# Hi-FT/ERD

Measured on AMD Instinct MI355X. Metric: images/sec GFL-R50 40+40 incre step @1333x800, higher is better.
Workload: dtype f32; 1 GPU; gfl_r50_fpn first_40_incre_last_40 ERD (BASELINE configs[1]), 1333x800 padded to 800x1344, fp32, procedural weights; batch_per_gpu=4, global_batch=4, parallelism=dp1

## Files before the change

erd_amd/_lib.py:

```python
from __future__ import annotations

import ctypes as C
import os

_HERE = os.path.dirname(os.path.abspath(__file__))
LIB_PATH = os.environ.get("ERD_HIP_LIB") or os.path.join(_HERE, "lib", "liberd_hip.so")

ERD_MAX_SEG = 5
ERD_MAX_TAPS = 9
ERD_MAX_GROUPS = 8
ERD_SQNORM_PARTS = 1024

c_float_p = C.c_void_p
i64 = C.c_int64
i32 = C.c_int
f32 = C.c_float


class ConvSeg(C.Structure):
    _fields_ = [("inp", C.c_void_p), ("out", C.c_void_p), ("res", C.c_void_p), ("alpha", C.c_void_p),
                ("mask", C.c_void_p), ("N", i32), ("IH", i32), ("IW", i32), ("GH", i32), ("GW", i32), ("OH", i32), ("OW", i32),
                ("in_nstride", i64), ("out_nstride", i64), ("res_nstride", i64),
                ("tap0", i32), ("ntaps", i32), ("oy", i32), ("ox", i32)]

# ... 64 lines not shown
    "erd_to_bf16": [P, P, i64, P],
    "erd_split3": [P, P, i64, P],
    "erd_conv_thin_enable": [i32],
    "erd_conv_thin_ok": [C.POINTER(ConvDesc)],
    "erd_weight_transpose_x3": [P, P, P, i32, i32, i32, i32, P],
    "erd_wino_weights_elems": [i32, i32],
    "erd_wino_weights": [P, P, i32, i32, i32, P],
    "erd_wino_conv3x3": [P, i32, P, i32, i32, P, P, i32, P, i32, P, P],
    "erd_wino_weights_x3_elems": [i32, i32],
    "erd_wino_weights_x3": [P, P, i32, i32, i32, P],
    "erd_wino_conv3x3_x3": [P, i32, P, i32, i32, P, P, i32, P, i32, P, P],
    "erd_wino_x3_couts_per_item": [P, i32, i32],
    "erd_wino_conv3x3_x3_gn": [P, i32, P, i32, i32, P, P, i32, P, P, C.c_size_t, P],
    "erd_wino_gn_finalize": [P, i32, i32, P, P, f32, P],
    "erd_wino_x3_gn_ws_bytes": [P, i32, i32],
    "erd_conv_wgrad": [C.POINTER(WgradDesc), P],
    "erd_wgrad_row3_slices": [C.POINTER(WgradDesc)],
    "erd_conv_grouped_fwd": [C.POINTER(ConvGroupedDesc), P],
    "erd_conv_grouped_dgrad": [C.POINTER(ConvGroupedDesc), P],
    "erd_conv_grouped_wgrad": [P, P, P, i32, i32, i32, i32, i32, i32, i32, P],
    "erd_conv_grouped_wgrad_splits": [i32, i32, i32, i32, i32, i32],
    "erd_deform_cols": [P, P, P, i32, i32, i32, i32, i32, P],
    "erd_deform_cols_bwd": [P, P, P, P, P, i32, i32, i32, i32, i32, P],
    "erd_wgrad_reduce": [P, i32, i32, i32, P, P, P, i32, P, P],
    "erd_wgrad_reduce_rows": [P, i32, i32, i32, i32, P, i32, P],
    "erd_wgrad_reduce_grouped": [P, i32, i32, i32, C.POINTER(WgradReduceGroups), i32, P],
    "erd_conv_wgrad_wino": [C.POINTER(WgradDesc), P],
    "erd_conv_wgrad_wino_ok": [C.POINTER(WgradDesc)],
    "erd_conv_wgrad_wino_tile": [C.POINTER(WgradDesc)],
    "erd_wgrad_wino_reduce": [P, i32, i32, i32, P, i32, P],
# ... 106 lines not shown
```

erd_amd/csrc/elementwise.hip:

```cpp
#include "erd_common.h"
#include <vector>

namespace erd {
thread_local char g_err[512] = "";
void set_error(const char* fmt, ...) {
    va_list ap;
    va_start(ap, fmt);
    vsnprintf(g_err, sizeof(g_err), fmt, ap);
    va_end(ap);
}
}

extern "C" int erd_abi_version(void) { return ERD_ABI_VERSION; }
#ifndef ERD_CSRC_SHA
#define ERD_CSRC_SHA "unknown"
#endif
extern "C" const char* erd_csrc_sha(void) { return ERD_CSRC_SHA; }
extern "C" __attribute__((weak)) int erd_probe_build_marker;
extern "C" int erd_probe_build(void) { return &erd_probe_build_marker != nullptr ? erd_probe_build_marker : 0; }
extern "C" const char* erd_last_error(void) { return erd::g_err; }
namespace erd {
static int g_cu_reserve = 0;
int usable_cus(int physical) { return physical - g_cu_reserve >= 8 ? physical - g_cu_reserve : (physical < 8 ? physical : 8); }
}
// ... 350 lines not shown
                                                       const float* __restrict__ gamma, const float* __restrict__ beta,
                                                       const float* __restrict__ mean_rstd, int64_t A, erd_levels lv,
                                                       GnChunks ch) {
    const int n = blockIdx.y;
    int s; int64_t r0, r1;
    gn_chunk(lv, ch, blockIdx.x, s, r0, r1);
    const int c4 = threadIdx.x & 63, rl = threadIdx.x >> 6;
    const int g = c4 >> 1;
    const float2 mr = *reinterpret_cast<const float2*>(mean_rstd + (((int64_t)n * lv.nseg + s) * G + g) * 2);
    const float4 ga = reinterpret_cast<const float4*>(gamma)[c4];
    const float4 be = reinterpret_cast<const float4*>(beta)[c4];
    for (int64_t r = r0 + rl; r < r1; r += 4) {
        const int64_t off = ((int64_t)n * A + r) * C + c4 * 4;
        const float4 v = erd::ld4(c + off);
        float4 o;
        o.x = fmaxf((v.x - mr.x) * mr.y * ga.x + be.x, 0.f);
        o.y = fmaxf((v.y - mr.x) * mr.y * ga.y + be.y, 0.f);
        o.z = fmaxf((v.z - mr.x) * mr.y * ga.z + be.z, 0.f);
        o.w = fmaxf((v.w - mr.x) * mr.y * ga.w + be.w, 0.f);
        erd::st4(y + off, o);
    }
}

template <int C, int G, typename T>
__global__ __launch_bounds__(256) void gn_bwd_stats_kernel(const T* __restrict__ c, const T* __restrict__ dy,
                                                           const float* __restrict__ gamma,
                                                           const float* __restrict__ beta,
                                                           const float* __restrict__ mean_rstd,
                                                           double* __restrict__ stats, float* __restrict__ dgamma,
                                                           float* __restrict__ dbeta, int64_t A, erd_levels lv,
                                                           GnChunks ch) {
    const int n = blockIdx.y;
    int s; int64_t r0, r1;
    gn_chunk(lv, ch, blockIdx.x, s, r0, r1, GN_STAT_ROWS);
// ... 844 lines not shown
```

erd_amd/csrc/erd_common.h:

```cpp
#pragma once
#include <hip/hip_runtime.h>
#include <stdint.h>
#include <stdio.h>
#include <stdarg.h>
#include "../../include/erd_hip.h"
#include "erd_probes.h"

namespace erd {

void set_error(const char* fmt, ...);
int usable_cus(int physical);

bool conv_thin_x3_ok(const erd_conv_desc* d);
int conv_thin_x3(const erd_conv_desc* d, hipStream_t st);
bool conv_thin_bf16_ok(const erd_conv_desc* d);
int conv_thin_bf16(const erd_conv_desc* d, hipStream_t st);

inline int check_launch(const char* what) {
    hipError_t e = hipGetLastError();
    if (e != hipSuccess) {
        set_error("%s: %s", what, hipGetErrorString(e));
        return (int)e;
    }
    return 0;
// ... 109 lines not shown
#pragma unroll
    for (int i = 0; i < 4; ++i) {
        const float u[4] = {t[i][0], 0.5f * (t[i][0] + t[i][1] + t[i][2]), 0.5f * (t[i][0] - t[i][1] + t[i][2]), t[i][2]};
#pragma unroll
        for (int j = 0; j < 4; ++j) {
            unsigned short hi, mid, lo;
            limbs3(u[j], hi, mid, lo);
            const int64_t o = (int64_t)((i * 4 + j) * 3) * per_xl + base;
            U3[o] = hi;
            U3[o + per_xl] = mid;
            U3[o + 2 * per_xl] = lo;
        }
    }
}

struct bf16s { unsigned short bits; };
__device__ __forceinline__ float4 ld4(const float* p) { return *reinterpret_cast<const float4*>(p); }
__device__ __forceinline__ float4 ld4(const bf16s* p) { return unpack4_bf16(*reinterpret_cast<const uint2*>(p)); }
__device__ __forceinline__ void st4(float* p, float4 v) { *reinterpret_cast<float4*>(p) = v; }
__device__ __forceinline__ void st4(bf16s* p, float4 v) { *reinterpret_cast<uint2*>(p) = pack4_bf16(v); }
__device__ __forceinline__ float ld1(const float* p) { return *p; }
__device__ __forceinline__ float ld1(const bf16s* p) { return __uint_as_float((unsigned)p->bits << 16); }
__device__ __forceinline__ void st1(float* p, float v) { *p = v; }
__device__ __forceinline__ void st1(bf16s* p, float v) { p->bits = (unsigned short)(pack2_bf16(v, 0.f) & 0xffffu); }

}
```

erd_amd/csrc/winograd.hip:

```cpp
#include "erd_common.h"
#include <type_traits>
#include <stdlib.h>
#include <algorithm>

namespace {

typedef float f32x4 __attribute__((ext_vector_type(4)));
typedef unsigned int u32x4 __attribute__((ext_vector_type(4)));
constexpr unsigned OOBV = 0x80000000u;

__device__ __forceinline__ float4 buf_load16_s(__amdgpu_buffer_rsrc_t r, unsigned voff, unsigned soff) {
    const u32x4 v = __builtin_amdgcn_raw_buffer_load_b128(r, voff, soff, 0);
    return make_float4(__uint_as_float(v.x), __uint_as_float(v.y), __uint_as_float(v.z), __uint_as_float(v.w));
}

constexpr int KS = 16;
constexpr int BN = 64;
constexpr int BNP = 128;
constexpr int RCS = 6;
#ifndef ERD_WINO_NCH
#define ERD_WINO_NCH 4
#endif
constexpr int NCH = ERD_WINO_NCH;
constexpr int MAXPIX = 64 * NCH;
// ... 985 lines not shown
        };
        if (t_half == 0) run(std::integral_constant<int, 0>{});
        else run(std::integral_constant<int, 1>{});
#ifdef ERD_WINO_TRACE
        if (wave == 0 && lane == 0 && blockIdx.x < 256) {
            g_wino_trace[blockIdx.x * 8 + 4] = __builtin_amdgcn_s_memtime() - t_begin;
            g_wino_trace[blockIdx.x * 8 + 5] = t_bar;
            g_wino_trace[blockIdx.x * 8 + 6] = t_ent;
            g_wino_trace[blockIdx.x * 8 + 7] = t_wait;
        }
#endif
    }
}

constexpr int HPIX = 208;

__global__ __launch_bounds__(512, 2) void wino_x3p_kernel(const WinoDesc p) {
    extern __shared__ __attribute__((aligned(16))) char smem[];
    constexpr unsigned RAWB = HPIX * RCS * 16, VOFF = 2 * RAWB, VB = VX_B, XOFF = VOFF + 2 * VB;
    float* sh_ss = reinterpret_cast<float*>(smem + XOFF);
    int* sh_item = reinterpret_cast<int*>(sh_ss + 4 * 2 * BNP);
    float* sh_gn = reinterpret_cast<float*>(sh_item + 4);
    char* const sm = smem;

    const int tid = threadIdx.x;
    const int Cin = p.Cin;
    const int nks = Cin / KS;
    const int nitems = p.nitems;
    const int ncb32 = (p.Cout + 31) / 32;
    int cur_item = blockIdx.x;


    const int wave = __builtin_amdgcn_readfirstlane(tid >> 6), lane = tid & 63;
    const int item0 = blockIdx.x;
    if (item0 >= nitems) return;

    const int li = lane & 31, h = lane >> 5;
// ... 16 lines not shown
    u32x4 ub[4][3];
    bf16x8 vf[2][3];
    auto load_u = [&](const int u, const unsigned soff) {
#pragma unroll
        for (int l = 0; l < 3; ++l)
            ub[u & 3][l] = __builtin_amdgcn_raw_buffer_load_b128(rs_U, u_lane, pos0_b + (unsigned)((u >> 1) * 3 + l) * per_xl_b + soff + (u & 1) * cb_b, 0);
    };

    WinoItem la = cur;
    int la_ks = 0, k_la = 0;
    unsigned la_soff = 0;
    bool la_valid = true;
    unsigned roff[2];
    float4 rv[2];
    __amdgpu_buffer_rsrc_t rs_in = __builtin_amdgcn_make_buffer_rsrc(const_cast<float*>(p.seg[0].in), 0, 0, 0x00020000);
    unsigned rdA = 0, rdB = 0, nrdA = 0, nrdB = 0;
    int tr_left = 0;
    auto item_geometry = [&](const WinoItem& it, unsigned (&ro)[2], unsigned& gA, unsigned& gB, __amdgpu_buffer_rsrc_t& rs) {
        const WinoSeg& sg = p.seg[it.s];
        rs = __builtin_amdgcn_make_buffer_rsrc(const_cast<float*>(sg.in), 0, (int)((long long)sg.N * sg.in_nstride * 4), 0x00020000);
        const int lbw = it.lbw, bw = 1 << lbw, bh = 32 >> lbw;
        const int pc_n = 2 * bw + 2, npix = (2 * bh + 2) * pc_n;
        const int recip = (65536 + pc_n - 1) / pc_n;
        const unsigned base_n = (unsigned)(it.n * sg.in_nstride);
#pragma unroll
        for (int i = 0; i < 2; ++i) {
            const int idx = tid + 512 * i;
            const int chunk = idx & 3, pix = idx >> 2;
            const int pr = (pix * recip) >> 16, pc = pix - pr * pc_n;
            const int iy = it.y0 - 1 + pr, ix = it.x0 - 1 + pc;
            ro[i] = OOBV;
            if (pix < npix && (unsigned)iy < (unsigned)sg.H && (unsigned)ix < (unsigned)sg.W)
                ro[i] = (base_n + (unsigned)((iy * sg.W + ix) * Cin + chunk * 4)) * 4u;
        }
        const int t_ty = t_tile >> lbw, t_tx = t_tile & (bw - 1);
        gA = (unsigned)((((2 * t_ty + rowA) * pc_n + 2 * t_tx) * RCS + t_chunk) * 16);
        gB = (unsigned)((((2 * t_ty + rowB) * pc_n + 2 * t_tx) * RCS + t_chunk) * 16);
    };
    struct Pending { float sc, sh; int claim, k; };
    auto request_item_data = [&](Pending& pe) {
        if (tid < BNP) {
            const int co = la.cout0 + tid;
            pe.sc = (p.scale && co < p.Cout) ? p.scale[co] : 1.f;
            pe.sh = (p.shift && co < p.Cout) ? p.shift[co] : 0.f;
        }
        if (tid == BNP) pe.claim = wino_claim(p, k_la);
        pe.k = k_la;
    };
    auto flush_pending = [&](const Pending& pe) {
        if (pe.k >= 0) {
            if (tid < BNP) {
                float* ss = sh_ss + (pe.k & 3) * (2 * BNP);
                ss[tid] = pe.sc;
                ss[BNP + tid] = pe.sh;
            }
            if (tid == BNP) sh_item[(pe.k + 1) & 1] = pe.claim;
        }
    };
    auto issue_next = [&](float4* dst) {
        if (la_valid) {
#pragma unroll
            for (int i = 0; i < 2; ++i) dst[i] = buf_load16_s(rs_in, roff[i], la_soff);
            la_soff += KS * 4;
            ++la_ks;
        }
    };
    auto advance_item = [&](Pending& pe) {
        if (la_valid && la_ks == nks) {
            const int nx = __builtin_amdgcn_readfirstlane(sh_item[(k_la + 1) & 1]);
            if (nx < nitems) {
                la = wino_decode<BNP>(p, nx);
                item_geometry(la, roff, nrdA, nrdB, rs_in);
                la_ks = 0;
                la_soff = 0;
                ++k_la;
                request_item_data(pe);
            } else la_valid = false;
        }
    };
    const bool st1_ok = (tid >> 2) + 128 < HPIX;
    auto store_raw = [&](const float4* src, const unsigned par) {
        int t = tid;
        asm volatile("" : "+v"(t));
        const unsigned st_base = (unsigned)(((t >> 2) * RCS + (t & 3)) * 16);
        *reinterpret_cast<float4*>(sm + par * RAWB + st_base) = src[0];
        if (st1_ok) *reinterpret_cast<float4*>(sm + par * RAWB + st_base + 128 * RCS * 16) = src[1];
    };
    float4 pd[2][4];
    auto transform_read = [&](const unsigned rpar) {
        const char* rA = sm + rpar * RAWB + rdA;
        const char* rB = sm + rpar * RAWB + rdB;
#pragma unroll
        for (int c = 0; c < 4; ++c) {
            pd[0][c] = *reinterpret_cast<const float4*>(rA + c * (RCS * 16));
            pd[1][c] = *reinterpret_cast<const float4*>(rB + c * (RCS * 16));
        }
        if (--tr_left == 0) {
            rdA = nrdA;
            rdB = nrdB;
            tr_left = nks;
        }
// ... 7 lines not shown
    auto row_pass = [&](float4 (&R)[4]) __attribute__((always_inline)) {
        if (t_row == 1) {
#pragma unroll
            for (int c = 0; c < 4; ++c) R[c] = f4add(pd[0][c], pd[1][c]);
        } else {
#pragma unroll
            for (int c = 0; c < 4; ++c) R[c] = f4sub(pd[0][c], pd[1][c]);
        }
    };
    unsigned long long t_d1 = 0, t_d2 = 0, t_d3 = 0, t_out = 0; (void)t_d1; (void)t_d2; (void)t_d3; (void)t_out;
    auto data_phase = [&](const unsigned par, const unsigned u_tail) __attribute__((always_inline)) {
        const unsigned npar = par ^ 1u;
        ERD_T0(ta);
        transform_read(npar);
        __builtin_amdgcn_sched_barrier(0);
        store_raw(rv, par);
#ifdef ERD_WINO_TRACE
        asm volatile("s_waitcnt lgkmcnt(0)" ::: "memory");
#endif
        ERD_TACC(t_d1, ta);
        ERD_T0(tb2);
        float4 R[4];
        row_pass(R);
        char* v = sm + v_write_base() + npar * VB;
        wino_put_limbs(v + 0 * 3072, f4sub(R[0], R[2]));
        wino_put_limbs(v + 1 * 3072, f4add(R[1], R[2]));
        wino_put_limbs(v + 2 * 3072, f4sub(R[2], R[1]));
        wino_put_limbs(v + 3 * 3072, f4sub(R[1], R[3]));
        __builtin_amdgcn_sched_barrier(0);
#ifdef ERD_WINO_TRACE
        asm volatile("s_waitcnt lgkmcnt(0)" ::: "memory");
#endif
        ERD_TACC(t_d2, tb2);
        ERD_T0(tc3);
        Pending pe;
        pe.sc = 1.f; pe.sh = 0.f; pe.claim = 0; pe.k = -1;
        advance_item(pe);
        flush_pending(pe);
        __builtin_amdgcn_sched_barrier(0);
        load_u(2, u_tail);
        load_u(3, u_tail);
        issue_next(rv);
        ERD_TACC(t_d3, tc3);
    };
    auto matrix_phase = [&](const unsigned par, const unsigned u_cur, const unsigned u_reload) __attribute__((always_inline)) {
        const char* vc = sm + VOFF + v_lane + par * VB;
#pragma unroll
        for (int l = 0; l < 3; ++l) vf[0][l] = *reinterpret_cast<const bf16x8*>(vc + l * 1024);
#pragma unroll
        for (int j = 0; j < 4; ++j) {
            if (j < 3) {
#pragma unroll
                for (int l = 0; l < 3; ++l) vf[(j + 1) & 1][l] = *reinterpret_cast<const bf16x8*>(vc + (j + 1) * 3072 + l * 1024);
            }
            __builtin_amdgcn_sched_barrier(0);
            const bf16x8 vh = vf[j & 1][0], vm = vf[j & 1][1], vl = vf[j & 1][2];
// ... 138 lines not shown
    };

    {
        float4 rvb[2];
#pragma unroll
        for (int i = 0; i < 2; ++i) { rv[i] = make_float4(0.f, 0.f, 0.f, 0.f); rvb[i] = rv[i]; }
        item_geometry(la, roff, nrdA, nrdB, rs_in);
        Pending pe;
        pe.sc = 1.f; pe.sh = 0.f; pe.claim = 0; pe.k = -1;
        request_item_data(pe);
        rdA = nrdA;
        rdB = nrdB;
        tr_left = nks;
        flush_pending(pe);
        pe.k = -1;
        issue_next(rv);
        issue_next(rvb);
#pragma unroll
        for (int q = 0; q < 4; ++q) load_u(q, u_item);
        store_raw(rv, 0);
        __syncthreads();
        transform_read(0);
        float4 R[4];
        row_pass(R);
        char* v = sm + v_write_base();
        wino_put_limbs(v + 0 * 3072, f4sub(R[0], R[2]));
        wino_put_limbs(v + 1 * 3072, f4add(R[1], R[2]));
        wino_put_limbs(v + 2 * 3072, f4sub(R[2], R[1]));
        wino_put_limbs(v + 3 * 3072, f4sub(R[1], R[3]));
        store_raw(rvb, 1);
        issue_next(rv);
        __syncthreads();
    }

    unsigned long long t_bar = 0, t_m = 0, t_d = 0; (void)t_bar; (void)t_m; (void)t_d;
    ERD_T0(t_begin);
    int g = 0;
    for (;;) {
        const int nxt_item = __builtin_amdgcn_readfirstlane(sh_item[(k_item + 1) & 1]);
        const bool has_next = nxt_item < nitems;
        const WinoItem nxt = has_next ? wino_decode<BNP>(p, nxt_item) : cur;
        const unsigned u_next = (unsigned)__builtin_amdgcn_readfirstlane(((nxt.cout0 >> 5) + 2 * cp) * nks * 1024);
#pragma unroll
        for (int q = 0; q < 8; ++q)
#pragma unroll
// ... 21 lines not shown
                tr[4] = t_d1;
                tr[5] = t_d2;
                tr[6] = t_d3;
                tr[7] = t_out;
            }
#endif
            if (tid == 0 && p.sched) wino_rearm(p);
            break;
        }
        cur = nxt;
        cur_item = nxt_item;
        u_item = u_next;
        ++k_item;
    }
}

__global__ __launch_bounds__(512) void wino_gn_finalize_kernel(const WinoDesc p, float* __restrict__ mean_rstd, float eps) {
    const int G = p.Cout >> 3;
    const int nb = blockIdx.x, s = blockIdx.y, n = blockIdx.z;
    if (n >= p.seg[s].N) return;
    const int q = threadIdx.x & 31, il = threadIdx.x >> 5;
    double acc = 0.0;
    for (int r = 0; r < p.nreg; ++r) {
        const WinoRegion& rg = p.reg[r];
        if (rg.seg != s) continue;
        const int per_img = rg.nby * rg.nbx;
        const int64_t it0 = (int64_t)nb * p.blocks_per_nb + rg.block0 + (int64_t)n * per_img;
        for (int b = il; b < per_img; b += 16) acc += (double)p.gn_part[(it0 + b) * 32 + q];
    }
    __shared__ double red[16][32];
// ... 99 lines not shown
        static int cached = 0;
        if (cached == 0 && hipGetDevice(&dev) == hipSuccess && hipGetDeviceProperties(&prop, dev) == hipSuccess)
            cached = prop.multiProcessorCount;
        ncu = erd::usable_cus(cached > 0 ? cached : 256);
    }
    const char* const e_mode = getenv("ERD_WINO_P");
    const int p_mode = e_mode ? atoi(e_mode) : 1;
    const int64_t i64 = (int64_t)blocks * ((Cout + BN - 1) / BN), i128 = (int64_t)blocks * (Cout / BNP);
    phased = x3 && p_mode != 0 && Cout % BNP == 0 && blocks > 0 &&
             (p_mode >= 2 || 16 * ((i128 + ncu - 1) / ncu) <= 10 * ((i64 + ncu - 1) / ncu));
    return 0;
}

int wino_launch(const erd_conv_seg* segs, int nseg, const float* U, const void* U3, int Cin, int Cout, const float* scale,
                const float* shift, int relu, float* colsum, int colsum_copies, int* sched, hipStream_t stream,
                float* gn_part = nullptr, size_t gn_part_bytes = 0) {
    ERD_REQUIRE(segs && (U || U3) && nseg >= 1 && nseg <= ERD_MAX_SEG, "wino: bad args");
    ERD_REQUIRE(Cin % KS == 0 && Cin >= 4 * KS && Cout > 0, "wino: Cin=%d must be a multiple of %d and at least %d", Cin, KS, 4 * KS);
    WinoDesc d;
    d.U = U;
    d.U3 = U3;
    d.Cin = Cin;
    d.Cout = Cout;
    d.scale = scale;
    d.shift = shift;
    d.relu = relu;
    d.colsum = colsum;
    ERD_REQUIRE(colsum_copies >= 0 && (colsum_copies & (colsum_copies - 1)) == 0, "wino: colsum_copies must be a power of two");
    d.colsum_copies = colsum_copies;
    d.sched = sched;
    d.gn_part = gn_part;
// ... 5 lines not shown
    if (blocks == 0) return 0;
    const int ncb = phased ? Cout / BNP : (Cout + BN - 1) / BN;
    d.nitems = blocks * ncb;
    static const int persist = getenv("ERD_WINO_PERSIST") ? atoi(getenv("ERD_WINO_PERSIST")) : 1;
    const int grid = persist ? (d.nitems < ncu ? d.nitems : ncu) : d.nitems;
    if (persist != 1) d.sched = nullptr;
    if (gn_part) {
        ERD_REQUIRE(Cout % 8 == 0, "wino: GroupNorm statistics need Cout %% 8 == 0");
        ERD_REQUIRE(phased && !colsum, "wino: the fused GroupNorm statistics need the 128-couts-per-item kernel (erd_wino_x3_couts_per_item) and no column sums");
        for (int q = 0; q < nseg; ++q) {
            ERD_REQUIRE(!segs[q].res && !segs[q].mask, "wino: the fused GroupNorm statistics serve plain convolutions (segment %d has a residual / mask)", q);
        }
        ERD_REQUIRE(gn_part_bytes >= (size_t)d.nitems * 32 * sizeof(float), "wino: GroupNorm partial-sum workspace too small (%zu bytes for %d items)",
                    gn_part_bytes, d.nitems);
    }
    if (phased) {
        const size_t lds = (size_t)2 * HPIX * RCS * 16 + 2 * VX_B + 4 * 2 * BNP * sizeof(float) + 16 + 4 * 16 * 2 * sizeof(float);
        static bool attrp_done = false;
        if (!attrp_done) {
            (void)hipFuncSetAttribute(reinterpret_cast<const void*>(wino_x3p_kernel), hipFuncAttributeMaxDynamicSharedMemorySize, (int)lds);
            attrp_done = true;
        }
        hipLaunchKernelGGL(wino_x3p_kernel, dim3((unsigned)grid), dim3(512), lds, stream, d);
        return erd::check_launch("wino_conv3x3_x3p");
    }
    if (U3) {
        const size_t lds = (size_t)2 * RAW_LDS_F4 * sizeof(float4) + 2 * VX_B + 4 * 2 * XCH_B + 64 + 2048 + 16;
        static bool attr3_done = false;
        if (!attr3_done) {
            (void)hipFuncSetAttribute(reinterpret_cast<const void*>(wino_x3_kernel), hipFuncAttributeMaxDynamicSharedMemorySize, (int)lds);
// ... 39 lines not shown
    return phased ? BNP : BN;
}

extern "C" int erd_wino_conv3x3_x3(const erd_conv_seg* segs, int nseg, const void* U3, int Cin, int Cout,
                                   const float* scale, const float* shift, int relu, float* colsum, int colsum_copies,
                                   int* sched, erd_stream_t stream) {
    ERD_REQUIRE(U3, "wino_x3: null U3");
    return wino_launch(segs, nseg, nullptr, U3, Cin, Cout, scale, shift, relu, colsum, colsum_copies, sched, (hipStream_t)stream);
}

extern "C" int erd_wino_conv3x3_x3_gn(const erd_conv_seg* segs, int nseg, const void* U3, int Cin, int Cout, const float* scale,
                                      const float* shift, int relu, int* sched, float* gn_part, size_t gn_part_bytes,
                                      erd_stream_t stream) {
    ERD_REQUIRE(U3 && gn_part, "wino_x3_gn: null U3 / gn_part");
    return wino_launch(segs, nseg, nullptr, U3, Cin, Cout, scale, shift, relu, nullptr, 0, sched, (hipStream_t)stream, gn_part, gn_part_bytes);
}

extern "C" int erd_wino_gn_finalize(const erd_conv_seg* segs, int nseg, int Cout, const float* gn_part, float* mean_rstd, float eps,
                                    erd_stream_t stream) {
    ERD_REQUIRE(segs && gn_part && mean_rstd && Cout % BNP == 0, "wino_gn_finalize: bad args");
    WinoDesc d;
    int ncu = 0, nmax = 0;
    bool phased = false;
    if (const int rc = wino_plan(d, segs, nseg, true, Cout, ncu, phased)) return rc;
    ERD_REQUIRE(phased, "wino_gn_finalize: these segments run on the 64-couts-per-item kernel (no partial sums exist)");
    d.Cout = Cout;
    d.gn_part = const_cast<float*>(gn_part);
    for (int q = 0; q < nseg; ++q) nmax = std::max(nmax, segs[q].N);
    hipLaunchKernelGGL(wino_gn_finalize_kernel, dim3((unsigned)(Cout / BNP), (unsigned)nseg, (unsigned)nmax), dim3(512), 0, (hipStream_t)stream, d,
                       mean_rstd, eps);
// ... 11 lines not shown
```

erd_amd/functional.py:

```python
from __future__ import annotations

from typing import List, Optional, Sequence, Tuple

import torch
from torch.autograd import Function

from . import kernels as K

Tensor = torch.Tensor


def ohwi(w: Tensor) -> Tensor:
    v = w.detach().permute(0, 2, 3, 1)
    if not v.is_contiguous():
        return v.contiguous()
    v._erd_owner = w
    return v


def _to_oihw(dw_ohwi: Tensor) -> Tensor:
    return dw_ohwi.permute(0, 3, 1, 2)


_AUX = {}
# ... 775 lines not shown
        if direct:
            _sunk(gamma)
            _sunk(beta)
            dgamma = dbeta = None
        wk = ohwi(w)
        dW = dx = None
        xv, dv = K.level_views(x_cat, sizes), K.level_views(dc, sizes)
        if ctx.needs_input_grad[1]:
            dW = _wgrad_plain(w, xv, dv, 3, 1, 1, keep=(x_cat, dc), trail=HEAD_TRAIL)
        if ctx.needs_input_grad[0]:
            dx = torch.empty_like(x_cat)
            K.conv_dgrad(dv, K.weight_transpose(wk), K.level_views(dx, sizes), 3, 1, 1)
        return dx, dW, dgamma, dbeta, None, None


class HeadConvBias(Function):

    @staticmethod
    def forward(ctx, x_cat, w, b, sizes):
        K.RECORDED = any(ctx.needs_input_grad)
        wk = ohwi(w)
        out = torch.empty((x_cat.shape[0], x_cat.shape[1], wk.shape[0]), dtype=torch.float32, device=x_cat.device)
        K.conv_forward(K.level_views(x_cat, sizes), wk, K.level_views(out, sizes), 3, 1, 1, shift=b.detach())
        ctx.sizes = sizes
        ctx.bias_param = b
        ctx.save_for_backward(x_cat, w)
        return out

    @staticmethod
    def backward(ctx, dy):
# ... 101 lines not shown
```

erd_amd/kernels.py:

```python
from __future__ import annotations

import ctypes as C
import os as _os
from typing import Dict, List, Optional, Sequence, Tuple

import torch

from . import _lib
from ._lib import ConvDesc, Levels, WgradDesc, call

Tensor = torch.Tensor


_raw_stream = getattr(torch._C, "_cuda_getCurrentRawStream", None)


def _cur_stream() -> int:
    if _raw_stream is not None:
        return _raw_stream(torch.cuda.current_device())
    return torch.cuda.current_stream().cuda_stream


def _stream() -> C.c_void_p:
    return C.c_void_p(_cur_stream())
# ... 1306 lines not shown
    U = _wino_weights_cached(w)
    lv = make_levels(sizes)
    part = workspace("gn_part", ws_bytes, c.device)
    mr = torch.empty((N, lv.nseg, G, 2), dtype=torch.float32, device=c.device)
    flop = 2.0 * N * A * Cout * 9 * Cin
    nbytes = (4.0 * (x_cat.numel() + c.numel()) + U.numel() * U.element_size()) if _TIMING is not None else 0.0
    _timed_call("conv_wino_fwd_p", flop, "erd_wino_conv3x3_x3_gn", segs, len(xs), _p(U), Cin, Cout, None, None, 0,
                _p(_wino_sched(U.device)), _p(part), ws_bytes, _stream(), nbytes=nbytes,
                tag=f"px{N * A} {Cin}->{Cout} k3s1" if TIMING_DETAIL else "")
    call("erd_wino_gn_finalize", segs, len(xs), Cout, _p(part), _p(mr), eps, _stream())
    y = torch.empty_like(c)
    call("erd_gn_relu_apply", _p(c), _p(y), _p(gamma), _p(beta), _p(mr), N, A, Cout, G, C.byref(lv), _mt(c), _stream())
    return c, y, mr


def gn_relu_backward(c: Tensor, dy: Tensor, gamma: Tensor, beta: Tensor, mr: Tensor, sizes, G: int = 32,
                     dgamma: Optional[Tensor] = None, dbeta: Optional[Tensor] = None):
    assert c.is_contiguous() and dy.is_contiguous()
    N, A, Cc = c.shape
    lv = make_levels(sizes)
    stats = workspace("gn_stats", N * lv.nseg * G * 16, c.device)
    dc = torch.empty_like(c)
    dgamma = zeros_f32(gamma.numel(), c.device) if dgamma is None else dgamma
    dbeta = zeros_f32(beta.numel(), c.device) if dbeta is None else dbeta
    call("erd_gn_relu_bwd", _p(c), _p(dy), _p(gamma), _p(beta), _p(mr), _p(stats), _p(dc), _p(dgamma), _p(dbeta), N, A,
         Cc, G, C.byref(lv), _mt(c, dy), _stream())
    return dc, dgamma, dbeta


def upsample_add_(fine: Tensor, coarse: Tensor) -> None:
# ... 329 lines not shown
```

erd_amd/modules.py:

```python
from __future__ import annotations

import math
import os
import sys
from collections import OrderedDict
from types import SimpleNamespace
from typing import Dict, List, Optional, Sequence, Tuple, Union

import numpy as np
import torch
import torch.nn as nn

from . import functional as Fn
from . import kernels as K
from .config import Config, ConfigDict
from .registry import MODELS, TASK_UTILS
from .structures import DetDataSample, InstanceData, unpack_gt_instances

Tensor = torch.Tensor


def _conv_weight(cout: int, cin: int, k: int) -> nn.Parameter:
    w = torch.empty((cout, k, k, cin), dtype=torch.float32).permute(0, 3, 1, 2)
    return nn.Parameter(w)
# ... 657 lines not shown
        self.gfl_cls = ConvHolder(256, self.cls_out_channels, 3, 1, 1, bias=True)
        self.gfl_reg = ConvHolder(256, 4 * (self.reg_max + 1), 3, 1, 1, bias=True)
        self.gfl_cls.reset_parameters("normal", 0.01, bias=float(-math.log((1 - 0.01) / 0.01)))
        self.gfl_reg.reset_parameters("normal", 0.01)
        self.scales = nn.ModuleList([Scale(1.0) for _ in self.prior_generator.strides])

    def forward_cat(self, p_cat: Tensor, sizes) -> Tuple[Tensor, Tensor]:
        _gpu_only(p_cat, "GFLHead.forward")
        sizes = [tuple(s) for s in sizes]
        cur = torch.cuda.current_stream(p_cat.device)
        aux = Fn.aux_stream(p_cat.device)
        forked = aux.cuda_stream != cur.cuda_stream
        if forked:
            aux.wait_stream(cur)
        with torch.cuda.stream(aux):
            r = p_cat
            for m in self.reg_convs:
                r = Fn.HeadConvGN.apply(r, m.conv.weight, m.gn.weight, m.gn.bias, sizes, m.gn.eps)
            pre = Fn.HeadConvBias.apply(r, self.gfl_reg.weight, self.gfl_reg.bias, sizes)
            alphas = torch.stack([s.scale for s in self.scales])
            bbox = Fn.LevelScale.apply(pre, alphas, sizes)
        c = p_cat
        for m in self.cls_convs:
            c = Fn.HeadConvGN.apply(c, m.conv.weight, m.gn.weight, m.gn.bias, sizes, m.gn.eps)
        cls = Fn.HeadConvBias.apply(c, self.gfl_cls.weight, self.gfl_cls.bias, sizes)
        if forked:
            cur.wait_stream(aux)
            bbox.record_stream(cur)
        return cls, bbox

    def forward(self, x: Sequence[Tensor]):
        sizes = [tuple(f.shape[-2:]) for f in x]
        cat = torch.cat([_nhwc(f).reshape(f.shape[0], -1, f.shape[1]) for f in x], 1)
        cls, bbox = self.forward_cat(cat, sizes)
        return ([_nchw(v) for v in K.level_views(cls, sizes)], [_nchw(v) for v in K.level_views(bbox, sizes)])

    def predict_by_feat_cat(self, cls: Tensor, bbox: Tensor, sizes, batch_img_metas, cfg=None, rescale: bool = False,
                            with_nms: bool = True) -> List[InstanceData]:
        _gpu_only(cls, "GFLHead.predict_by_feat")
# ... 520 lines not shown
```

include/erd_hip.h:

```cpp
#ifndef ERD_HIP_H_
#define ERD_HIP_H_

#include <stddef.h>
#include <stdint.h>

#ifdef __cplusplus
extern "C" {
#endif

#define ERD_ABI_VERSION 6
#define ERD_MAX_SEG 5
#define ERD_MAX_TAPS 9
#define ERD_MAX_GROUPS 8

#define ERD_EINVAL (-1)
#define ERD_EUNSUPPORTED (-2)

typedef void* erd_stream_t;

enum { ERD_F32 = 0, ERD_BF16 = 1 };

int erd_abi_version(void);
int erd_set_cu_reserve(int n);
int erd_usable_cus(void);
// ... 45 lines not shown
int erd_wino_conv3x3(const erd_conv_seg* segs, int nseg, const float* U, int Cin, int Cout, const float* scale,
                     const float* shift, int relu, float* colsum, int colsum_copies ,
                     int* sched ,
                     erd_stream_t stream);

size_t erd_wino_weights_x3_elems(int Cout, int Cin);
int erd_wino_weights_x3(const float* w_ohwi, void* U3, int Cout, int Cin, int flip, erd_stream_t stream);
int erd_wino_conv3x3_x3(const erd_conv_seg* segs, int nseg, const void* U3, int Cin, int Cout, const float* scale,
                        const float* shift, int relu, float* colsum, int colsum_copies, int* sched, erd_stream_t stream);
int erd_wino_x3_couts_per_item(const erd_conv_seg* segs, int nseg, int Cout);
int erd_wino_conv3x3_x3_gn(const erd_conv_seg* segs, int nseg, const void* U3, int Cin, int Cout, const float* scale,
                           const float* shift, int relu, int* sched, float* gn_part, size_t gn_part_bytes, erd_stream_t stream);
int erd_wino_gn_finalize(const erd_conv_seg* segs, int nseg, int Cout, const float* gn_part, float* mean_rstd, float eps,
                         erd_stream_t stream);
size_t erd_wino_x3_gn_ws_bytes(const erd_conv_seg* segs, int nseg, int Cout);

typedef struct {
    int64_t x_off, dz_off;
    int N, IH, IW, GH, GW, OH, OW;
    int64_t x_nstride, dz_nstride;
} erd_wgrad_seg;

typedef struct {
    const float* x;
    const float* dz;
    int64_t x_elems, dz_elems;
    int nseg;
    erd_wgrad_seg seg[ERD_MAX_SEG];
    int Cin, Cout, ntaps;
    int dy[ERD_MAX_TAPS], dx[ERD_MAX_TAPS];
// ... 258 lines not shown
```

Baseline: 129.8 images/sec.

## Fuse GroupNorm+ReLU of previous tower layer into Winograd conv input load

Adds a templated Winograd 3x3 kernel variant that applies the previous layer's GroupNorm affine and ReLU while staging raw input tiles into LDS. The head towers now chain conv-with-stats calls instead of separate conv, GN stats and GN apply passes. This removes a standalone full read and write of each intermediate activation. In training it still writes the normalized activation back from LDS for the backward pass, which adds stores, extra LDS and some register pressure inside the conv kernel.

```diff
diff --git a/erd_amd/_lib.py b/erd_amd/_lib.py
--- a/erd_amd/_lib.py
+++ b/erd_amd/_lib.py
@@ -102,6 +102,8 @@
     "erd_wino_conv3x3_x3_gn": [P, i32, P, i32, i32, P, P, i32, P, P, C.c_size_t, P],
     "erd_wino_gn_finalize": [P, i32, i32, P, P, f32, P],
     "erd_wino_x3_gn_ws_bytes": [P, i32, i32],
+    "erd_wino_x3_gn_in_ok": [P, i32, i32, i32],
+    "erd_wino_conv3x3_x3_gn_in": [P, i32, P, i32, i32, P, P, i32, P, P, C.c_size_t, P, P, P, P, P],
     "erd_conv_wgrad": [C.POINTER(WgradDesc), P],
     "erd_wgrad_row3_slices": [C.POINTER(WgradDesc)],
     "erd_conv_grouped_fwd": [C.POINTER(ConvGroupedDesc), P],
diff --git a/erd_amd/csrc/elementwise.hip b/erd_amd/csrc/elementwise.hip
--- a/erd_amd/csrc/elementwise.hip
+++ b/erd_amd/csrc/elementwise.hip
@@ -388,10 +388,10 @@
         const int64_t off = ((int64_t)n * A + r) * C + c4 * 4;
         const float4 v = erd::ld4(c + off);
         float4 o;
-        o.x = fmaxf((v.x - mr.x) * mr.y * ga.x + be.x, 0.f);
-        o.y = fmaxf((v.y - mr.x) * mr.y * ga.y + be.y, 0.f);
-        o.z = fmaxf((v.z - mr.x) * mr.y * ga.z + be.z, 0.f);
-        o.w = fmaxf((v.w - mr.x) * mr.y * ga.w + be.w, 0.f);
+        o.x = erd::gn_relu_value(v.x, mr.x, mr.y, ga.x, be.x);
+        o.y = erd::gn_relu_value(v.y, mr.x, mr.y, ga.y, be.y);
+        o.z = erd::gn_relu_value(v.z, mr.x, mr.y, ga.z, be.z);
+        o.w = erd::gn_relu_value(v.w, mr.x, mr.y, ga.w, be.w);
         erd::st4(y + off, o);
     }
 }
diff --git a/erd_amd/csrc/erd_common.h b/erd_amd/csrc/erd_common.h
--- a/erd_amd/csrc/erd_common.h
+++ b/erd_amd/csrc/erd_common.h
@@ -147,6 +147,16 @@
     }
 }
 
+__device__ __forceinline__ float gn_affine(float c, float mean, float rstd, float gamma, float beta) {
+    return __builtin_fmaf(gamma, (c - mean) * rstd, beta);
+}
+__device__ __forceinline__ float gn_relu_value(float c, float mean, float rstd, float gamma, float beta) {
+    return fmaxf(gn_affine(c, mean, rstd, gamma, beta), 0.f);
+}
+__device__ __forceinline__ float gn_relu_value_or_zero(float c, float mean, float rstd, float gamma, float beta, float hi) {
+    return __builtin_amdgcn_fmed3f(gn_affine(c, mean, rstd, gamma, beta), 0.f, hi);
+}
+
 struct bf16s { unsigned short bits; };
 __device__ __forceinline__ float4 ld4(const float* p) { return *reinterpret_cast<const float4*>(p); }
 __device__ __forceinline__ float4 ld4(const bf16s* p) { return unpack4_bf16(*reinterpret_cast<const uint2*>(p)); }
diff --git a/erd_amd/csrc/winograd.hip b/erd_amd/csrc/winograd.hip
--- a/erd_amd/csrc/winograd.hip
+++ b/erd_amd/csrc/winograd.hip
@@ -1023,13 +1023,25 @@
 }
 
 constexpr int HPIX = 208;
-
-__global__ __launch_bounds__(512, 2) void wino_x3p_kernel(const WinoDesc p) {
+constexpr int GN_IN_C = 256, GN_IN_G = 32;
+
+struct WinoGnIn {
+    const float* mean_rstd;
+    const float* gamma;
+    const float* beta;
+    float* y[ERD_MAX_SEG];
+};
+
+template <bool GNIN>
+__device__ __forceinline__ void wino_x3p_body(const WinoDesc& p, const WinoGnIn& gi) {
     extern __shared__ __attribute__((aligned(16))) char smem[];
     constexpr unsigned RAWB = HPIX * RCS * 16, VOFF = 2 * RAWB, VB = VX_B, XOFF = VOFF + 2 * VB;
     float* sh_ss = reinterpret_cast<float*>(smem + XOFF);
     int* sh_item = reinterpret_cast<int*>(sh_ss + 4 * 2 * BNP);
     float* sh_gn = reinterpret_cast<float*>(sh_item + 4);
+    float* sh_gb = sh_gn + 4 * 16 * 2;
+    float* sh_mr = sh_gb + 2 * GN_IN_C;
+    constexpr unsigned GBOFF = XOFF + 4 * 2 * BNP * 4 + 16 + 4 * 16 * 2 * 4, MROFF = GBOFF + 2 * GN_IN_C * 4;
     char* const sm = smem;
 
     const int tid = threadIdx.x;
@@ -1076,6 +1088,9 @@
     unsigned roff[2];
     float4 rv[2];
     __amdgpu_buffer_rsrc_t rs_in = __builtin_amdgcn_make_buffer_rsrc(const_cast<float*>(p.seg[0].in), 0, 0, 0x00020000);
+    unsigned woff[2] = {OOBV, OOBV};
+    __amdgpu_buffer_rsrc_t rs_y = rs_in;
+    bool wb_on = false, rv_new = false;
     unsigned rdA = 0, rdB = 0, nrdA = 0, nrdB = 0;
     int tr_left = 0;
     auto item_geometry = [&](const WinoItem& it, unsigned (&ro)[2], unsigned& gA, unsigned& gB, __amdgpu_buffer_rsrc_t& rs) {
@@ -1094,17 +1109,29 @@
             ro[i] = OOBV;
             if (pix < npix && (unsigned)iy < (unsigned)sg.H && (unsigned)ix < (unsigned)sg.W)
                 ro[i] = (base_n + (unsigned)((iy * sg.W + ix) * Cin + chunk * 4)) * 4u;
+            if constexpr (GNIN) {
+                const bool own = pix < npix && pr >= 1 && pr <= 2 * bh && pc >= 1 && pc <= 2 * bw && iy < it.yl && ix < it.xl;
+                woff[i] = own ? ro[i] : OOBV;
+            }
+        }
+        if constexpr (GNIN) {
+            float* const yp = gi.y[it.s];
+            wb_on = yp != nullptr && it.cout0 == 0;
+            rs_y = __builtin_amdgcn_make_buffer_rsrc(yp, 0, yp ? (int)((long long)sg.N * sg.in_nstride * 4) : 0, 0x00020000);
         }
         const int t_ty = t_tile >> lbw, t_tx = t_tile & (bw - 1);
         gA = (unsigned)((((2 * t_ty + rowA) * pc_n + 2 * t_tx) * RCS + t_chunk) * 16);
         gB = (unsigned)((((2 * t_ty + rowB) * pc_n + 2 * t_tx) * RCS + t_chunk) * 16);
     };
-    struct Pending { float sc, sh; int claim, k; };
+    struct Pending { float sc, sh; int claim, k; float mr; };
     auto request_item_data = [&](Pending& pe) {
         if (tid < BNP) {
             const int co = la.cout0 + tid;
             pe.sc = (p.scale && co < p.Cout) ? p.scale[co] : 1.f;
             pe.sh = (p.shift && co < p.Cout) ? p.shift[co] : 0.f;
+        }
+        if constexpr (GNIN) {
+            if (tid >= 256 && tid < 256 + 2 * GN_IN_G) pe.mr = gi.mean_rstd[(la.n * p.nseg + la.s) * (2 * GN_IN_G) + (tid - 256)];
         }
         if (tid == BNP) pe.claim = wino_claim(p, k_la);
         pe.k = k_la;
@@ -1117,9 +1144,13 @@
                 ss[BNP + tid] = pe.sh;
             }
             if (tid == BNP) sh_item[(pe.k + 1) & 1] = pe.claim;
+            if constexpr (GNIN) {
+                if (tid >= 256 && tid < 256 + 2 * GN_IN_G) sh_mr[(pe.k & 1) * (2 * GN_IN_G) + (tid - 256)] = pe.mr;
+            }
         }
     };
     auto issue_next = [&](float4* dst) {
+        if constexpr (GNIN) rv_new = la_valid;
         if (la_valid) {
 #pragma unroll
             for (int i = 0; i < 2; ++i) dst[i] = buf_load16_s(rs_in, roff[i], la_soff);
@@ -1141,12 +1172,41 @@
         }
     };
     const bool st1_ok = (tid >> 2) + 128 < HPIX;
-    auto store_raw = [&](const float4* src, const unsigned par) {
+    auto store_raw = [&](const float4* src, const unsigned par, const unsigned soff) {
         int t = tid;
         asm volatile("" : "+v"(t));
         const unsigned st_base = (unsigned)(((t >> 2) * RCS + (t & 3)) * 16);
+        if constexpr (GNIN) {
+            const unsigned c16 = (unsigned)(t & 3) * 16u;
+            const float4 ga = *reinterpret_cast<const float4*>(sm + GBOFF + soff + c16);
+            const float4 be = *reinterpret_cast<const float4*>(sm + GBOFF + GN_IN_C * 4 + soff + c16);
+            const float2 mr = *reinterpret_cast<const float2*>(sm + MROFF + (unsigned)(k_la & 1) * (2 * GN_IN_G * 4) + (soff >> 2) + ((c16 >> 5) << 3));
+            float4 yv[2];
+#pragma unroll
+            for (int i = 0; i < 2; ++i) {
+                const float hi = roff[i] == OOBV ? 0.f : __builtin_inff();
+                yv[i].x = erd::gn_relu_value_or_zero(src[i].x, mr.x, mr.y, ga.x, be.x, hi);
+                yv[i].y = erd::gn_relu_value_or_zero(src[i].y, mr.x, mr.y, ga.y, be.y, hi);
+                yv[i].z = erd::gn_relu_value_or_zero(src[i].z, mr.x, mr.y, ga.z, be.z, hi);
+                yv[i].w = erd::gn_relu_value_or_zero(src[i].w, mr.x, mr.y, ga.w, be.w, hi);
+            }
+            *reinterpret_cast<float4*>(sm + par * RAWB + st_base) = yv[0];
+            if (st1_ok) *reinterpret_cast<float4*>(sm + par * RAWB + st_base + 128 * RCS * 16) = yv[1];
+            return;
+        }
         *reinterpret_cast<float4*>(sm + par * RAWB + st_base) = src[0];
         if (st1_ok) *reinterpret_cast<float4*>(sm + par * RAWB + st_base + 128 * RCS * 16) = src[1];
+    };
+    [[maybe_unused]] auto write_back = [&](const unsigned par, const unsigned soff) {
+        if (wb_on && rv_new) {
+            int t = tid;
+            asm volatile("" : "+v"(t));
+            const unsigned st_base = (unsigned)(((t >> 2) * RCS + (t & 3)) * 16);
+            const u32x4 a = *reinterpret_cast<const u32x4*>(sm + par * RAWB + st_base);
+            const u32x4 b = *reinterpret_cast<const u32x4*>(sm + par * RAWB + st_base + (st1_ok ? 128 * RCS * 16 : 0));
+            __builtin_amdgcn_raw_buffer_store_b128(a, rs_y, woff[0], soff, 0);
+            __builtin_amdgcn_raw_buffer_store_b128(b, rs_y, woff[1], soff, 0);
+        }
     };
     float4 pd[2][4];
     auto transform_read = [&](const unsigned rpar) {
@@ -1184,7 +1244,7 @@
         ERD_T0(ta);
         transform_read(npar);
         __builtin_amdgcn_sched_barrier(0);
-        store_raw(rv, par);
+        store_raw(rv, par, la_soff - KS * 4);
 #ifdef ERD_WINO_TRACE
         asm volatile("s_waitcnt lgkmcnt(0)" ::: "memory");
 #endif
@@ -1205,11 +1265,19 @@
         ERD_T0(tc3);
         Pending pe;
         pe.sc = 1.f; pe.sh = 0.f; pe.claim = 0; pe.k = -1;
+        if constexpr (GNIN) {
+            load_u(2, u_tail);
+            load_u(3, u_tail);
+            write_back(par, la_soff - KS * 4);
+            __builtin_amdgcn_sched_barrier(0);
+        }
         advance_item(pe);
         flush_pending(pe);
         __builtin_amdgcn_sched_barrier(0);
-        load_u(2, u_tail);
-        load_u(3, u_tail);
+        if constexpr (!GNIN) {
+            load_u(2, u_tail);
+            load_u(3, u_tail);
+        }
         issue_next(rv);
         ERD_TACC(t_d3, tc3);
     };
@@ -1378,11 +1446,14 @@
         tr_left = nks;
         flush_pending(pe);
         pe.k = -1;
+        if constexpr (GNIN) sh_gb[tid] = tid < GN_IN_C ? gi.gamma[tid] : gi.beta[tid - GN_IN_C];
         issue_next(rv);
         issue_next(rvb);
 #pragma unroll
         for (int q = 0; q < 4; ++q) load_u(q, u_item);
-        store_raw(rv, 0);
+        if constexpr (GNIN) __syncthreads();
+        store_raw(rv, 0, 0);
+        if constexpr (GNIN) write_back(0, 0);
         __syncthreads();
         transform_read(0);
         float4 R[4];
@@ -1392,7 +1463,8 @@
         wino_put_limbs(v + 1 * 3072, f4add(R[1], R[2]));
         wino_put_limbs(v + 2 * 3072, f4sub(R[2], R[1]));
         wino_put_limbs(v + 3 * 3072, f4sub(R[1], R[3]));
-        store_raw(rvb, 1);
+        store_raw(rvb, 1, KS * 4);
+        if constexpr (GNIN) write_back(1, KS * 4);
         issue_next(rv);
         __syncthreads();
     }
@@ -1444,6 +1516,16 @@
         ++k_item;
     }
 }
+
+__global__ __launch_bounds__(512, 2) void wino_x3p_kernel(const WinoDesc p) {
+    WinoGnIn none;
+    wino_x3p_body<false>(p, none);
+}
+struct WinoDescIn {
+    WinoDesc d;
+    WinoGnIn gn;
+};
+__global__ __launch_bounds__(512, 2) void wino_x3p_in_kernel(const WinoDescIn p) { wino_x3p_body<true>(p.d, p.gn); }
 
 __global__ __launch_bounds__(512) void wino_gn_finalize_kernel(const WinoDesc p, float* __restrict__ mean_rstd, float eps) {
     const int G = p.Cout >> 3;
@@ -1573,7 +1655,7 @@
 
 int wino_launch(const erd_conv_seg* segs, int nseg, const float* U, const void* U3, int Cin, int Cout, const float* scale,
                 const float* shift, int relu, float* colsum, int colsum_copies, int* sched, hipStream_t stream,
-                float* gn_part = nullptr, size_t gn_part_bytes = 0) {
+                float* gn_part = nullptr, size_t gn_part_bytes = 0, const WinoGnIn* gn_in = nullptr) {
     ERD_REQUIRE(segs && (U || U3) && nseg >= 1 && nseg <= ERD_MAX_SEG, "wino: bad args");
     ERD_REQUIRE(Cin % KS == 0 && Cin >= 4 * KS && Cout > 0, "wino: Cin=%d must be a multiple of %d and at least %d", Cin, KS, 4 * KS);
     WinoDesc d;
@@ -1609,6 +1691,22 @@
         ERD_REQUIRE(gn_part_bytes >= (size_t)d.nitems * 32 * sizeof(float), "wino: GroupNorm partial-sum workspace too small (%zu bytes for %d items)",
                     gn_part_bytes, d.nitems);
     }
+    if (gn_in) {
+        ERD_REQUIRE(phased, "wino: the on-load GroupNorm needs the 128-couts-per-item kernel (erd_wino_x3_gn_in_ok)");
+        ERD_REQUIRE(Cin == GN_IN_C, "wino: the on-load GroupNorm is built for Cin = %d with %d groups (Cin=%d)", GN_IN_C, GN_IN_G, Cin);
+        WinoDescIn di;
+        di.d = d;
+        di.gn = *gn_in;
+        const size_t lds = (size_t)2 * HPIX * RCS * 16 + 2 * VX_B + 4 * 2 * BNP * sizeof(float) + 16 + 4 * 16 * 2 * sizeof(float) +
+                           2 * GN_IN_C * sizeof(float) + 2 * 2 * GN_IN_G * sizeof(float);
+        static bool attri_done = false;
+        if (!attri_done) {
+            (void)hipFuncSetAttribute(reinterpret_cast<const void*>(wino_x3p_in_kernel), hipFuncAttributeMaxDynamicSharedMemorySize, (int)lds);
+            attri_done = true;
+        }
+        hipLaunchKernelGGL(wino_x3p_in_kernel, dim3((unsigned)grid), dim3(512), lds, stream, di);
+        return erd::check_launch("wino_conv3x3_x3p_in");
+    }
     if (phased) {
         const size_t lds = (size_t)2 * HPIX * RCS * 16 + 2 * VX_B + 4 * 2 * BNP * sizeof(float) + 16 + 4 * 16 * 2 * sizeof(float);
         static bool attrp_done = false;
@@ -1678,6 +1776,34 @@
                                       erd_stream_t stream) {
     ERD_REQUIRE(U3 && gn_part, "wino_x3_gn: null U3 / gn_part");
     return wino_launch(segs, nseg, nullptr, U3, Cin, Cout, scale, shift, relu, nullptr, 0, sched, (hipStream_t)stream, gn_part, gn_part_bytes);
+}
+
+extern "C" int erd_wino_x3_gn_in_ok(const erd_conv_seg* segs, int nseg, int Cin, int Cout) {
+    WinoDesc d;
+    int ncu = 0;
+    bool phased = false;
+    if (!segs || Cin != GN_IN_C || Cout <= 0 || wino_plan(d, segs, nseg, true, Cout, ncu, phased) != 0) return 0;
+    return phased ? 1 : 0;
+}
+
+extern "C" int erd_wino_conv3x3_x3_gn_in(const erd_conv_seg* segs, int nseg, const void* U3, int Cin, int Cout, const float* scale,
+                                         const float* shift, int relu, int* sched, float* gn_part, size_t gn_part_bytes,
+                                         const float* in_mean_rstd, const float* in_gamma, const float* in_beta, float* const* in_y,
+                                         erd_stream_t stream) {
+    ERD_REQUIRE(U3 && segs && in_mean_rstd && in_gamma && in_beta, "wino_x3_gn_in: null U3 / segs / mean_rstd / gamma / beta");
+    ERD_REQUIRE(nseg >= 1 && nseg <= ERD_MAX_SEG, "wino_x3_gn_in: bad segment count %d", nseg);
+    ERD_REQUIRE(Cin == GN_IN_C, "wino_x3_gn_in: only Cin = %d with %d groups is built (Cin=%d)", GN_IN_C, GN_IN_G, Cin);
+    ERD_REQUIRE(erd_wino_x3_gn_in_ok(segs, nseg, Cin, Cout) == 1,
+                "wino_x3_gn_in: this launch runs on the 64-couts-per-item kernel (erd_wino_x3_gn_in_ok)");
+    WinoGnIn g;
+    g.mean_rstd = in_mean_rstd;
+    g.gamma = in_gamma;
+    g.beta = in_beta;
+    for (int q = 0; q < ERD_MAX_SEG; ++q) g.y[q] = (in_y && q < nseg) ? in_y[q] : nullptr;
+    for (int q = 0; q < nseg; ++q) {
+        ERD_REQUIRE(!g.y[q] || (g.y[q] != segs[q].in && g.y[q] != segs[q].out), "wino_x3_gn_in: segment %d writes y over its input / output", q);
+    }
+    return wino_launch(segs, nseg, nullptr, U3, Cin, Cout, scale, shift, relu, nullptr, 0, sched, (hipStream_t)stream, gn_part, gn_part_bytes, &g);
 }
 
 extern "C" int erd_wino_gn_finalize(const erd_conv_seg* segs, int nseg, int Cout, const float* gn_part, float* mean_rstd, float eps,
diff --git a/erd_amd/functional.py b/erd_amd/functional.py
--- a/erd_amd/functional.py
+++ b/erd_amd/functional.py
@@ -813,6 +813,102 @@
         return dx, dW, dgamma, dbeta, None, None
 
 
+def _tower_conv_backward(ctx, x_in, w, dc, sizes, need_dx: bool):
+    wk = ohwi(w)
+    dW = dx = None
+    xv, dv = K.level_views(x_in, sizes), K.level_views(dc, sizes)
+    if ctx.needs_input_grad[ctx.w_index]:
+        dW = _wgrad_plain(w, xv, dv, 3, 1, 1, keep=(x_in, dc), trail=HEAD_TRAIL)
+    if need_dx:
+        dx = torch.empty_like(x_in)
+        K.conv_dgrad(dv, K.weight_transpose(wk), K.level_views(dx, sizes), 3, 1, 1)
+    return dx, dW
+
+
+def _gn_backward(c, dy, gamma, beta, mr, sizes):
+    gs, bs_ = _sink(gamma), _sink(beta)
+    direct = gs is not None and bs_ is not None
+    dc, dgamma, dbeta = K.gn_relu_backward(c, dy.contiguous(), gamma.detach(), beta.detach(), mr, sizes, 32,
+                                           dgamma=gs if direct else None, dbeta=bs_ if direct else None)
+    if direct:
+        _sunk(gamma)
+        _sunk(beta)
+        dgamma = dbeta = None
+    return dc, dgamma, dbeta
+
+
+class HeadConvStats(Function):
+
+    @staticmethod
+    def forward(ctx, x_cat, w, sizes, eps: float):
+        K.RECORDED = any(ctx.needs_input_grad)
+        c, mr, _ = K.conv3x3_gn_stats_forward(x_cat, ohwi(w), sizes, eps)
+        ctx.sizes, ctx.w_index = sizes, 1
+        ctx.save_for_backward(x_cat, w)
+        ctx.mark_non_differentiable(mr)
+        return c, mr
+
+    @staticmethod
+    def backward(ctx, dc, _dmr):
+        x_cat, w = ctx.saved_tensors
+        dx, dW = _tower_conv_backward(ctx, x_cat, w, dc.contiguous(), ctx.sizes, ctx.needs_input_grad[0])
+        return dx, dW, None, None
+
+
+class HeadGNConvStats(Function):
+
+    @staticmethod
+    def forward(ctx, c_prev, mr_prev, gamma, beta, w, sizes, eps: float):
+        K.RECORDED = any(ctx.needs_input_grad)
+        c, mr, y_prev = K.conv3x3_gn_stats_forward(c_prev, ohwi(w), sizes, eps, gn_in=(mr_prev, gamma.detach(), beta.detach()),
+                                                   want_y=K.RECORDED)
+        ctx.sizes, ctx.w_index = sizes, 4
+        ctx.save_for_backward(c_prev, mr_prev, gamma, beta, w, y_prev)
+        ctx.mark_non_differentiable(mr)
+        return c, mr
+
+    @staticmethod
+    def backward(ctx, dc, _dmr):
+        c_prev, mr_prev, gamma, beta, w, y_prev = ctx.saved_tensors
+        sizes = ctx.sizes
+        need_dy = ctx.needs_input_grad[0] or ctx.needs_input_grad[2] or ctx.needs_input_grad[3]
+        dy_prev, dW = _tower_conv_backward(ctx, y_prev, w, dc.contiguous(), sizes, need_dy)
+        dc_prev = dgamma = dbeta = None
+        if need_dy:
+            dc_prev, dgamma, dbeta = _gn_backward(c_prev, dy_prev, gamma, beta, mr_prev, sizes)
+        return dc_prev, None, dgamma, dbeta, dW, None, None
+
+
+class HeadGNApply(Function):
+
+    @staticmethod
+    def forward(ctx, c, mr, gamma, beta, sizes):
+        y = K.gn_relu_apply(c, mr, gamma.detach(), beta.detach(), sizes, 32)
+        ctx.sizes = sizes
+        ctx.save_for_backward(c, mr, gamma, beta)
+        return y
+
+    @staticmethod
+    def backward(ctx, dy):
+        c, mr, gamma, beta = ctx.saved_tensors
+        dc, dgamma, dbeta = _gn_backward(c, dy, gamma, beta, mr, ctx.sizes)
+        return dc, None, dgamma, dbeta, None
+
+
+def head_tower(x_cat, convs, sizes):
+    convs = list(convs)
+    K.RECORDED = torch.is_grad_enabled() and (x_cat.requires_grad or any(p.requires_grad for m in convs for p in (m.conv.weight, m.gn.weight, m.gn.bias)))
+    if len(convs) < 2 or not all(tuple(m.conv.weight.shape) == (256, 256, 3, 3) for m in convs) or \
+            not K.gn_onload_ok(x_cat, 256, sizes):
+        for m in convs:
+            x_cat = HeadConvGN.apply(x_cat, m.conv.weight, m.gn.weight, m.gn.bias, sizes, m.gn.eps)
+        return x_cat
+    c, mr = HeadConvStats.apply(x_cat, convs[0].conv.weight, sizes, convs[0].gn.eps)
+    for prev, m in zip(convs[:-1], convs[1:]):
+        c, mr = HeadGNConvStats.apply(c, mr, prev.gn.weight, prev.gn.bias, m.conv.weight, sizes, m.gn.eps)
+    return HeadGNApply.apply(c, mr, convs[-1].gn.weight, convs[-1].gn.bias, sizes)
+
+
 class HeadConvBias(Function):
 
     @staticmethod
diff --git a/erd_amd/kernels.py b/erd_amd/kernels.py
--- a/erd_amd/kernels.py
+++ b/erd_amd/kernels.py
@@ -1344,6 +1344,73 @@
     return c, y, mr
 
 
+GN_ONLOAD = _os.environ.get("ERD_GN_ONLOAD", "1") != "0"
+
+
+def _tower_segs(x_cat: Tensor, c: Tensor, sizes):
+    from ._lib import ConvSeg
+    xs, outs = level_views(x_cat, sizes), level_views(c, sizes)
+    segs = (ConvSeg * len(xs))()
+    for i, (x, o) in enumerate(zip(xs, outs)):
+        _fill_seg(segs[i], x, o, x.shape[1], x.shape[2], None, None, None)
+    return segs, len(xs)
+
+
+def gn_onload_ok(x_cat: Tensor, Cout: int, sizes, G: int = 32) -> bool:
+    if not (GN_ONLOAD and GN_FUSED and x_cat.is_cuda and x_cat.dtype == torch.float32 and x_cat.dim() == 3 and x_cat.is_contiguous()):
+        return False
+    N, A, Cin = x_cat.shape
+    if not (Cin == 256 and Cout == 256 and G == 32 and wino_ok(Cin, 3, 1, 1) and wino_x3()):
+        return False
+    if not (WINO_TRAIN_FWD if RECORDED else WINO_NOGRAD_FWD) or torch.cuda.is_current_stream_capturing():
+        return False
+    segs, n = _tower_segs(x_cat, x_cat, sizes)
+    return int(_lib.load().erd_wino_x3_gn_in_ok(segs, n, Cin, Cout)) == 1
+
+
+def conv3x3_gn_stats_forward(x_cat: Tensor, w: Tensor, sizes, eps: float = 1e-5, gn_in=None, want_y: bool = False):
+    _require_gpu(x_cat, w)
+    N, A, Cin = x_cat.shape
+    Cout = w.shape[0]
+    c = torch.empty((N, A, Cout), dtype=x_cat.dtype, device=x_cat.device)
+    segs, n = _tower_segs(x_cat, c, sizes)
+    ws_bytes = int(_lib.load().erd_wino_x3_gn_ws_bytes(segs, n, Cout))
+    if ws_bytes == 0:
+        raise _lib.ErdHipError("conv3x3_gn_stats_forward: this launch runs on the 64-couts-per-item kernel (check gn_onload_ok first)")
+    U = _wino_weights_cached(w)
+    part = workspace("gn_part", ws_bytes, c.device)
+    mr = torch.empty((N, n, Cout // 8, 2), dtype=torch.float32, device=c.device)
+    flop = 2.0 * N * A * Cout * 9 * Cin
+    nbytes = (4.0 * (x_cat.numel() + c.numel()) + U.numel() * U.element_size()) if _TIMING is not None else 0.0
+    tag = f"px{N * A} {Cin}->{Cout} k3s1" if TIMING_DETAIL else ""
+    y_in = None
+    if gn_in is None:
+        _timed_call("conv_wino_fwd_p", flop, "erd_wino_conv3x3_x3_gn", segs, n, _p(U), Cin, Cout, None, None, 0,
+                    _p(_wino_sched(U.device)), _p(part), ws_bytes, _stream(), nbytes=nbytes, tag=tag)
+    else:
+        in_mr, in_gamma, in_beta = gn_in
+        assert in_mr.shape == (N, n, Cin // 8, 2) and in_mr.is_contiguous() and in_gamma.numel() == Cin and in_beta.numel() == Cin
+        yp = None
+        if want_y:
+            y_in = torch.empty_like(x_cat)
+            yp = (C.c_void_p * n)(*[v.data_ptr() for v in level_views(y_in, sizes)])
+        _timed_call("conv_wino_fwd_p", flop, "erd_wino_conv3x3_x3_gn_in", segs, n, _p(U), Cin, Cout, None, None, 0,
+                    _p(_wino_sched(U.device)), _p(part), ws_bytes, _p(in_mr), _p(in_gamma), _p(in_beta), yp, _stream(),
+                    nbytes=nbytes + (4.0 * x_cat.numel() if want_y and _TIMING is not None else 0.0), tag=tag)
+    call("erd_wino_gn_finalize", segs, n, Cout, _p(part), _p(mr), eps, _stream())
+    return c, mr, y_in
+
+
+def gn_relu_apply(c: Tensor, mr: Tensor, gamma: Tensor, beta: Tensor, sizes, G: int = 32) -> Tensor:
+    _require_gpu(c)
+    assert c.is_contiguous()
+    N, A, Cc = c.shape
+    lv = make_levels(sizes)
+    y = torch.empty_like(c)
+    call("erd_gn_relu_apply", _p(c), _p(y), _p(gamma), _p(beta), _p(mr), N, A, Cc, G, C.byref(lv), _mt(c), _stream())
+    return y
+
+
 def gn_relu_backward(c: Tensor, dy: Tensor, gamma: Tensor, beta: Tensor, mr: Tensor, sizes, G: int = 32,
                      dgamma: Optional[Tensor] = None, dbeta: Optional[Tensor] = None):
     assert c.is_contiguous() and dy.is_contiguous()
diff --git a/erd_amd/modules.py b/erd_amd/modules.py
--- a/erd_amd/modules.py
+++ b/erd_amd/modules.py
@@ -695,15 +695,11 @@
         if forked:
             aux.wait_stream(cur)
         with torch.cuda.stream(aux):
-            r = p_cat
-            for m in self.reg_convs:
-                r = Fn.HeadConvGN.apply(r, m.conv.weight, m.gn.weight, m.gn.bias, sizes, m.gn.eps)
+            r = Fn.head_tower(p_cat, self.reg_convs, sizes)
             pre = Fn.HeadConvBias.apply(r, self.gfl_reg.weight, self.gfl_reg.bias, sizes)
             alphas = torch.stack([s.scale for s in self.scales])
             bbox = Fn.LevelScale.apply(pre, alphas, sizes)
-        c = p_cat
-        for m in self.cls_convs:
-            c = Fn.HeadConvGN.apply(c, m.conv.weight, m.gn.weight, m.gn.bias, sizes, m.gn.eps)
+        c = Fn.head_tower(p_cat, self.cls_convs, sizes)
         cls = Fn.HeadConvBias.apply(c, self.gfl_cls.weight, self.gfl_cls.bias, sizes)
         if forked:
             cur.wait_stream(aux)
diff --git a/include/erd_hip.h b/include/erd_hip.h
--- a/include/erd_hip.h
+++ b/include/erd_hip.h
@@ -83,6 +83,11 @@
 int erd_wino_gn_finalize(const erd_conv_seg* segs, int nseg, int Cout, const float* gn_part, float* mean_rstd, float eps,
                          erd_stream_t stream);
 size_t erd_wino_x3_gn_ws_bytes(const erd_conv_seg* segs, int nseg, int Cout);
+int erd_wino_x3_gn_in_ok(const erd_conv_seg* segs, int nseg, int Cin, int Cout);
+int erd_wino_conv3x3_x3_gn_in(const erd_conv_seg* segs, int nseg, const void* U3, int Cin, int Cout, const float* scale,
+                              const float* shift, int relu, int* sched, float* gn_part, size_t gn_part_bytes,
+                              const float* in_mean_rstd, const float* in_gamma, const float* in_beta, float* const* in_y,
+                              erd_stream_t stream);
 
 typedef struct {
     int64_t x_off, dz_off;
```

After: 130.6 images/sec (median of 6 runs). Within noise of the previous version (+0.6%).
